# sisinflab/elliot

Measured on NVIDIA H100. Metric: bpr_triples_per_sec, higher is better.
Workload: dtype f32

## Files before the change

### elliot_b200/_lib.py

```python
import ctypes
import os

_HERE = os.path.dirname(os.path.abspath(__file__))
LIB_PATH = os.path.join(_HERE, "csrc", "libelliot_b200.so")

c_i32, c_i64, c_u64, c_f32, c_f64 = ctypes.c_int32, ctypes.c_int64, ctypes.c_uint64, ctypes.c_float, ctypes.c_double
c_int, c_void, c_size = ctypes.c_int, ctypes.c_void_p, ctypes.c_size_t

SIGNATURES = {
    "eb_last_error": (ctypes.c_char_p, []),
    "eb_version": (c_int, []),
    "eb_device_info": (c_int, [c_void, c_void]),
    "eb_bpr_step_f32": (c_int, [c_void, c_void, c_void, c_int, c_int, c_void, c_void, c_void, c_i64,
                                c_f32, c_f32, c_f32, c_f32, c_f32, c_void, c_int, c_void]),
    "eb_bpr_step_sampled_f32": (c_int, [c_void, c_void, c_void, c_int, c_int, c_i32, c_i32, c_void, c_void,
                                        c_i64, c_u64, c_u64, c_f32, c_f32, c_f32, c_f32, c_f32,
                                        c_void, c_void, c_void, c_void, c_void, c_size, c_int, c_void]),
    "eb_bpr_step_sampled_workspace_bytes": (c_size, [c_i64, c_i32]),
    "eb_bloom_build": (c_int, [c_void, c_void, c_i32, c_int, c_void, c_void]),
    "eb_bpr_step_sampled_filter_f32": (c_int, [c_void, c_void, c_void, c_int, c_int, c_i32, c_i32, c_void, c_void, c_void, c_int,
                                               c_i64, c_u64, c_u64, c_f32, c_f32, c_f32, c_f32, c_f32,
                                               c_void, c_void, c_void, c_void, c_void, c_size, c_int, c_void]),
    "eb_bpr_sample_philox_filter": (c_int, [c_i32, c_i32, c_void, c_void, c_void, c_int, c_i64, c_u64, c_u64, c_void, c_void, c_void,
                                            c_void]),
    "eb_bpr_sample_philox": (c_int, [c_i32, c_i32, c_void, c_void, c_i64, c_u64, c_u64, c_void, c_void, c_void,
                                     c_void]),
    "eb_bpr_step_host_f32": (c_int, [c_void, c_void, c_void, c_int, c_int, c_void, c_void, c_void, c_i64,
                                     c_f32, c_f32, c_f32, c_f32, c_f32, c_void, c_void, c_void, c_int, c_void]),
    "eb_bpr_step_host_packed_f32": (c_int, [c_void, c_void, c_void, c_int, c_int, c_void, c_i64, c_int, c_int,
                                            c_f32, c_f32, c_f32, c_f32, c_f32, c_void, c_void, c_void, c_int, c_void]),
    "eb_bpr_exact_workspace_bytes": (c_size, [c_i64, c_i32, c_i32]),
    "eb_bpr_exact_f64": (c_int, [c_void, c_void, c_void, c_int, c_int, c_i32, c_i32, c_void, c_void, c_void, c_i64,
                                 c_f64, c_f64, c_f64, c_f64, c_f64, c_void, c_void, c_size, c_void]),
    "eb_mt_seed": (c_int, [c_void, ctypes.c_uint32, c_void]),
    "eb_mt_sampler_workspace_bytes": (c_size, [c_i64]),
    "eb_mt_sampler_step": (c_int, [c_void, c_i32, c_i32, c_void, c_void, c_void, c_i64, c_void, c_void, c_void,
                                   c_void, c_size, c_void]),
    "eb_mt_raw": (c_int, [c_void, c_void, c_i64, c_void]),
    "eb_score_topk_workspace_bytes": (c_size, [c_i64, c_i32, c_int]),
    "eb_score_topk_f32": (c_int, [c_void, c_void, c_void, c_i32, c_int, c_int, c_void, c_void, c_void, c_i32, c_i64,
                                  c_int, c_void, c_void, c_void, c_size, c_void]),
    "eb_score_topk_f64": (c_int, [c_void, c_void, c_void, c_i32, c_int, c_int, c_void, c_void, c_void, c_i32, c_i64,
                                  c_int, c_void, c_void, c_void, c_size, c_void]),
    "eb_bpr_batch_grad_f32": (c_int, [c_void, c_void, c_void, c_void, c_void, c_void, c_int, c_int, c_void, c_void, c_void,
                                      c_i64, c_f32, c_f32, c_void, c_void]),
    "eb_adam_dense_f32": (c_int, [c_void, c_void, c_void, c_void, c_i64, c_f32, c_f32, c_f32, c_f32, c_i64, c_void]),
    "eb_adam_dense_copy_f32": (c_int, [c_void, c_void, c_void, c_void, c_i64, c_f32, c_f32, c_f32, c_f32, c_i64, c_void, c_void]),
    "eb_convert_bf16": (c_int, [c_void, c_int, c_int, c_i64, c_void, c_i64, c_int, c_void]),
    "eb_gemm_bf16_tn": (c_int, [c_void, c_i64, c_void, c_i64, c_void, c_i64, c_int, c_int, c_int, c_void, c_f32, c_int,
                                c_void]),
    "eb_gemm_bf16": (c_int, [c_void, c_i64, c_int, c_void, c_i64, c_int, c_void, c_i64, c_int, c_int, c_int, c_void, c_f32, c_int,
                             c_void]),
    "eb_gemm_bf16_out": (c_int, [c_void, c_i64, c_int, c_void, c_i64, c_int, c_void, c_i64, c_void, c_i64, c_int, c_int, c_int, c_void,
                                 c_f32, c_int, c_void]),
    "eb_gemm_f32_ref": (c_int, [c_void, c_i64, c_int, c_void, c_i64, c_int, c_void, c_i64, c_int, c_int, c_int, c_void, c_f32, c_int,
                                c_void]),
    "eb_vae_embed_fwd": (c_int, [c_void, c_void, c_int, c_void, c_void, c_void, c_int, c_void, c_i64, c_f32, c_u64, c_void]),
    "eb_vae_embed_bwd": (c_int, [c_void, c_int, c_void, c_void, c_void, c_int, c_void, c_i64, c_f32, c_u64, c_void]),
    "eb_vae_reparam_fwd": (c_int, [c_void, c_i64, c_int, c_int, c_void, c_i64, c_u64, c_u64, c_void, c_void]),
    "eb_vae_reparam_bwd": (c_int, [c_void, c_i64, c_int, c_int, c_void, c_i64, c_void, c_i64, c_u64, c_u64, c_f32, c_void]),
    "eb_vae_softmax": (c_int, [c_void, c_i64, c_int, c_void, c_void, c_void, c_int, c_void, c_void, c_int, c_void]),
    "eb_vae_softmax_bf16": (c_int, [c_void, c_i64, c_int, c_void, c_void, c_void, c_int, c_void, c_void, c_int, c_void, c_i64, c_void]),
    "eb_tanh_bwd": (c_int, [c_void, c_void, c_void, c_i64, c_void]),
    "eb_colsum": (c_int, [c_void, c_int, c_int, c_i64, c_void, c_void]),
    "eb_dense_topk_f32": (c_int, [c_void, c_i64, c_int, c_int, c_void, c_void, c_void, c_void, c_int, c_void, c_void, c_void]),
    "eb_neumf_gather": (c_int, [c_void, c_void, c_void, c_void, c_int, c_i64, c_void, c_void, c_i64, c_void, c_i64, c_void, c_i64, c_void]),
    "eb_neumf_head": (c_int, [c_void, c_i64, c_void, c_i64, c_int, c_void, c_void, c_void, c_i64, c_void, c_void, c_void, c_void,
                              c_void, c_void, c_void]),
    "eb_neumf_head_norm": (c_int, [c_void, c_i64, c_void, c_i64, c_int, c_void, c_void, c_void, c_i64, c_i64, c_void, c_void, c_void,
                                   c_void, c_void, c_void, c_void]),
    "eb_relu_bwd_copy": (c_int, [c_void, c_void, c_void, c_i64, c_void, c_void]),
    "eb_relu_bwd": (c_int, [c_void, c_void, c_void, c_i64, c_void]),
    "eb_neumf_scatter": (c_int, [c_void, c_void, c_int, c_i64, c_void, c_void, c_i64, c_void, c_i64, c_void, c_i64, c_void, c_void,
                                 c_void, c_void, c_void]),
    "eb_neumf_sample": (c_int, [c_i32, c_i32, c_void, c_void, c_int, c_u64, c_i64, c_void, c_void, c_void, c_void]),
    "eb_neumf_pair_h1": (c_int, [c_void, c_i64, c_void, c_i64, c_void, c_int, c_int, c_int, c_void, c_i64, c_void]),
    "eb_neumf_pair_h1_f32": (c_int, [c_void, c_i64, c_void, c_i64, c_void, c_int, c_int, c_int, c_void, c_i64, c_void]),
    "eb_neumf_pair_head": (c_int, [c_void, c_void, c_i64, c_int, c_int, c_int, c_int, c_void, c_i64, c_void, c_void, c_void, c_i64,
                                   c_void]),
    "eb_gather_rows_f32": (c_int, [c_void, c_i64, c_void, c_i64, c_int, c_void, c_i64, c_void]),
    "eb_scatter_add_rows_f32": (c_int, [c_void, c_i64, c_void, c_i64, c_int, c_void, c_i64, c_void]),
    "eb_bpr_step_rows_f32": (c_int, [c_void, c_i64, c_void, c_void, c_void, c_i64, c_i64, c_int, c_f32, c_f32, c_f32, c_f32, c_f32,
                                     c_void, c_void, c_void, c_void]),
    "eb_table_delta_f32": (c_int, [c_void, c_void, c_void, c_i64, c_void]),
    "eb_table_apply_delta_f32": (c_int, [c_void, c_void, c_void, c_i64, c_f32, c_void]),
    "eb_vae_step_workspace_bytes": (c_size, [c_int, c_int, c_int, c_int]),
    "eb_vae_train_step": (c_int, [c_void, c_void, c_int, c_f32, c_u64, c_u64, c_u64, c_f32, c_f32, c_void, c_void, c_size, c_int, c_void]),
    "eb_mf_pointwise_exact_f64": (c_int, [c_void, c_void, c_void, c_void, c_void, c_int, c_int, c_void, c_void, c_void, c_i64,
                                  c_f64, c_f64, c_i64, c_void, c_void]),
    "eb_mf_pointwise_step_f32": (c_int, [c_void, c_void, c_void, c_void, c_void, c_int, c_int, c_void, c_void, c_i64, c_int, c_i32,
                                 c_u64, c_u64, c_i64, c_i64, c_f32, c_f32, c_void, c_void, c_void, c_void, c_void, c_void]),
    "eb_eval_topk_workspace_bytes": (c_size, [c_i64, c_int]),
    "eb_eval_topk_f64": (c_int, [c_void, c_i64, c_int, c_int, c_void, c_void, c_void, c_void, c_void, c_void, c_void, c_void,
                         c_void, c_size, c_void]),
    "eb_partition_streams_create": (c_int, [c_int, c_int, ctypes.POINTER(ctypes.c_void_p), ctypes.POINTER(c_int)]),
    "eb_table_apply_delta_late_f32": (c_int, [c_void, c_void, c_void, c_void, c_i64, c_f32, c_void]),
    "eb_gmf_step_grads": (c_int, [c_void, c_void, c_i64, c_int, c_void, c_void, c_void, c_void, c_i64, c_i64, c_void, c_void, c_void,
                                  c_void, c_void]),
    "eb_gmf_scale_rows": (c_int, [c_void, c_i64, c_i64, c_int, c_void, c_void, c_i64, c_void]),
    "eb_sigmoid_inplace": (c_int, [c_void, c_i64, c_void]),
    "eb_pointwise_sample_philox": (c_int, [c_i32, c_i32, c_void, c_void, c_void, c_int, c_i64, c_u64, c_u64, c_void, c_void, c_void,
                                           c_void]),
    "eb_peer_alloc": (c_int, [c_size, ctypes.POINTER(ctypes.c_void_p)]),
    "eb_peer_free": (c_int, [c_void]),
    "eb_peer_export": (c_int, [c_void, c_void]),
# ... 81 lines not shown
```

### elliot_b200/csrc/bpr_train.cu

```cuda
#include <cooperative_groups.h>
#include <cub/cub.cuh>
#include <stdlib.h>

#include <type_traits>

#include "bpr_update.cuh"

namespace eb {

struct HogwildParams {
    float *U, *V, *b;
    int ld;
    const int32_t *tu, *ti, *tj;
    int64_t n;
    BprHyper hp;
    double *loss;
    int32_t n_users, n_items;
    const int64_t *indptr;
    const int32_t *indices;
    uint64_t seed, first;
    int32_t *out_u, *out_i, *out_j;
    float *Vp[EB_MAX_PEERS], *bp[EB_MAX_PEERS];
    ShardMap shards;
    const uint32_t *filter;
// ... 529 lines not shown

template <int DP, bool SAMPLE, bool ATOMIC, bool PEER, bool ROUNDS>
static int launch_hogwild_t(const HogwildParams &p, int reserve_sms, cudaStream_t st) {
    auto kern = bpr_hogwild_kernel<DP, SAMPLE, ATOMIC, PEER, ROUNDS>;
    unsigned grid;
    if (int rc = persistent_grid((const void *)kern, 0, p.n, reserve_sms, grid)) return rc;
    if (ROUNDS) {
        void *args[] = {const_cast<HogwildParams *>(&p)};
        EB_CUDA(cudaLaunchCooperativeKernel((const void *)kern, dim3(grid), dim3(256), args, 0, st));
    } else {
        kern<<<grid, 256, 0, st>>>(p);
    }
    EB_CUDA(cudaGetLastError());
    return EB_OK;
}

template <int... DPS, class F>
static int with_stride(int dp, const char *strides, F &&f) {
    int rc = EB_OK;
    const bool found = ((dp == DPS && (rc = f(std::integral_constant<int, DPS>{}), true)) || ...);
    return found ? rc : set_err(EB_ERR_ARG, "row stride ld=%d must be one of %s", dp, strides);
}

static void item_table_l2_window(const HogwildParams &p, cudaStream_t st) {
    static const int env = [] { const char *e = getenv("EB_L2_PERSIST"); return e ? atoi(e) : 0; }();
    if (!env || !p.V) return;
    static int max_persist = -1, max_window = 0;
    if (max_persist < 0) {
        int dev = 0; cudaGetDevice(&dev);
        cudaDeviceGetAttribute(&max_persist, cudaDevAttrMaxPersistingL2CacheSize, dev);
        cudaDeviceGetAttribute(&max_window, cudaDevAttrMaxAccessPolicyWindowSize, dev);
    }
    const size_t bytes = (size_t)p.n_items * (size_t)p.ld * sizeof(float);
    if (max_persist <= 0 || bytes > (size_t)max_persist || bytes > (size_t)max_window) return;
    static size_t carved = 0;
    if (carved != bytes) { cudaDeviceSetLimit(cudaLimitPersistingL2CacheSize, bytes); carved = bytes; }
    cudaStreamAttrValue attr{};
    attr.accessPolicyWindow.base_ptr = (void *)p.V;
    attr.accessPolicyWindow.num_bytes = bytes;
    attr.accessPolicyWindow.hitRatio = 1.0f;
    attr.accessPolicyWindow.hitProp = cudaAccessPropertyPersisting;
    attr.accessPolicyWindow.missProp = env == 2 ? cudaAccessPropertyNormal : cudaAccessPropertyStreaming;
    cudaStreamSetAttribute(st, cudaStreamAttributeAccessPolicyWindow, &attr);
}

template <int DP, bool ATOMIC>
static int launch_grouped_t(const HogwildParams &p, int reserve_sms, cudaStream_t st) {
    auto kern = bpr_grouped_kernel<DP, ATOMIC>;
    unsigned grid;
    if (int rc = persistent_grid((const void *)kern, 0, p.n, reserve_sms, grid)) return rc;
    kern<<<grid, 256, 0, st>>>(p);
    EB_CUDA(cudaGetLastError());
    return EB_OK;
}

static inline size_t align_up(size_t x, size_t a = 256) { return (x + a - 1) / a * a; }

static int bits_for(uint64_t v) { int b = 1; while ((v >> b) != 0) b++; return b; }

constexpr int64_t GROUP_MAX = (int64_t)INT32_MAX;

struct GroupLayout {
    size_t key_a, key_b, val_a, val_b, cub, cub_bytes, total;
};

static GroupLayout group_layout(int64_t n, int32_t n_users) {
    const int64_t m = n < GROUP_MAX ? n : GROUP_MAX;
    GroupLayout L;
    size_t off = 0;
    L.key_a = off; off += align_up(sizeof(uint32_t) * (size_t)m);
    L.key_b = off; off += align_up(sizeof(uint32_t) * (size_t)m);
    L.val_a = off; off += align_up(sizeof(int32_t) * (size_t)m);
    L.val_b = off; off += align_up(sizeof(int32_t) * (size_t)m);
    cub::DoubleBuffer<uint32_t> keys(nullptr, nullptr);
    cub::DoubleBuffer<int32_t> vals(nullptr, nullptr);
    size_t cb = 0;
    cub::DeviceRadixSort::SortPairs(nullptr, cb, keys, vals, (int)m, 0, bits_for((uint64_t)n_users));
    L.cub_bytes = cb;
    L.cub = off; off += align_up(cb);
    L.total = off;
    return L;
}

template <int DP, bool ATOMIC>
static int launch_grouped(HogwildParams p, int reserve, char *ws, const GroupLayout &L, cudaStream_t st) {
    const int ubits = bits_for((uint64_t)p.n_users);
    const int64_t n = p.n;
    const uint64_t first = p.first;
    int32_t *out_u = p.out_u, *out_i = p.out_i, *out_j = p.out_j;
    int sms = sm_count() - reserve;
    if (sms < 1) sms = 1;
    for (int64_t c0 = 0; c0 < n; c0 += GROUP_MAX) {
        p.n = n - c0 < GROUP_MAX ? n - c0 : GROUP_MAX;
        p.first = first + (uint64_t)c0;
        if (out_u) { p.out_u = out_u + c0; p.out_i = out_i + c0; p.out_j = out_j + c0; }
        cub::DoubleBuffer<uint32_t> keys((uint32_t *)(ws + L.key_a), (uint32_t *)(ws + L.key_b));
        cub::DoubleBuffer<int32_t> vals((int32_t *)(ws + L.val_a), (int32_t *)(ws + L.val_b));
        int64_t grid = (p.n + 255) / 256;
        if (grid > (int64_t)sms * 8) grid = (int64_t)sms * 8;
        user_key_kernel<<<(unsigned)grid, 256, 0, st>>>(p, keys.Current(), vals.Current());
        EB_CUDA(cudaGetLastError());
        size_t cb = L.cub_bytes;
        EB_CUDA(cub::DeviceRadixSort::SortPairs(ws + L.cub, cb, keys, vals, (int)p.n, 0, ubits, st));
        p.order = vals.Current();
        if (int rc = launch_grouped_t<DP, ATOMIC>(p, reserve, st)) return rc;
    }
    return EB_OK;
}

template <bool SAMPLE>
static int launch_hogwild(const HogwildParams &p, int dp, int flags, cudaStream_t st, void *ws = nullptr, size_t ws_bytes = 0) {
    const bool atomic = !(flags & 1);
    const bool rounds = (flags & 64) != 0;
    const int reserve = (flags >> 8) & 0xff;
    EB_ARG(!(flags & 32), "the shared-memory-staged kernel exists for sharded item tables only");
    EB_ARG(atomic || !rounds, "deterministic rounds run with atomic updates");
    if constexpr (SAMPLE) {
        if (!rounds) {
            const GroupLayout L = group_layout(p.n, p.n_users);
            if (!ws || ws_bytes < L.total) return set_err(EB_ERR_WORKSPACE, "workspace %zu < required %zu", ws ? ws_bytes : 0, L.total);
            return with_stride<8, 16, 32, 64, 128, 256>(dp, "8,16,32,64,128,256 floats", [&](auto dpc) {
                constexpr int DP = decltype(dpc)::value;
                item_table_l2_window(p, st);
                return atomic ? launch_grouped<DP, true>(p, reserve, (char *)ws, L, st)
                              : launch_grouped<DP, false>(p, reserve, (char *)ws, L, st);
            });
        }
    }
    item_table_l2_window(p, st);
    return with_stride<8, 16, 32, 64, 128, 256>(dp, "8,16,32,64,128,256 floats", [&](auto dpc) {
        constexpr int DP = decltype(dpc)::value;
        if constexpr (!SAMPLE) {
            if (!rounds) return atomic ? launch_hogwild_t<DP, false, true, false, false>(p, reserve, st)
                                       : launch_hogwild_t<DP, false, false, false, false>(p, reserve, st);
        }
        return launch_hogwild_t<DP, SAMPLE, true, false, true>(p, reserve, st);
    });
}

template <bool SAMPLE>
static int launch_hogwild_peer(const HogwildParams &p, int dp, int flags, cudaStream_t st) {
    const int reserve = (flags >> 8) & 0xff;
    EB_ARG(!(flags & 64), "deterministic rounds exist for local tables only (other GPUs update peer rows concurrently)");
    const bool stage = !(flags & (1 | 16));
    return with_stride<32, 64, 128>(dp, "32,64,128 floats for sharded item tables", [&](auto dpc) {
        constexpr int DP = decltype(dpc)::value;
        return stage ? launch_stage_t<DP, SAMPLE>(p, reserve, st) : launch_hogwild_t<DP, SAMPLE, true, true, false>(p, reserve, st);
    });
}

static int fill_peer(HogwildParams &p, float *const *V_shards, float *const *b_shards, int n_shards, int32_t shard_rows,
                     int32_t n_items) {
    EB_ARG(V_shards && b_shards && n_shards >= 1 && n_shards <= EB_MAX_PEERS, "1 <= n_shards <= %d", EB_MAX_PEERS);
    EB_ARG(shard_rows >= 1 && (int64_t)shard_rows * n_shards >= n_items, "shards do not cover the item range");
    for (int s = 0; s < n_shards; s++) {
        EB_ARG(V_shards[s] && b_shards[s] && ((uintptr_t)V_shards[s] % 16) == 0, "null / misaligned shard pointer %d", s);
        p.Vp[s] = V_shards[s]; p.bp[s] = b_shards[s];
    }
    for (int s = n_shards; s < EB_MAX_PEERS; s++) { p.Vp[s] = V_shards[0]; p.bp[s] = b_shards[0]; }
    p.shards = shard_map(shard_rows);
    return EB_OK;
}

static int check_tables(const void *U, const void *V, const void *b, int d, int ld) {
    EB_ARG(U && V && b, "null table pointer");
    EB_ARG(d >= 1 && ld >= d, "need 1 <= d <= ld (d=%d ld=%d)", d, ld);
    EB_ARG(((uintptr_t)U % 16) == 0 && ((uintptr_t)V % 16) == 0, "tables must be 16-byte aligned");
    return EB_OK;
}

struct ExactParams {
    double *U, *V, *b;
    int d, ld;
    const int32_t *tu, *ti, *tj;
    const int32_t *ku, *ki, *kj;
    int32_t *cntU, *cntI, *ticket;
    int64_t n;
    double lr, reg_u, reg_b, reg_pos, reg_neg;
    double *loss;
};

__device__ __forceinline__ int ld_acquire(const int32_t *p) {
    int v;
    asm volatile("ld.acquire.gpu.global.s32 %0, [%1];" : "=r"(v) : "l"(p) : "memory");
    return v;
}
__device__ __forceinline__ void st_release(int32_t *p, int v) {
    asm volatile("st.release.gpu.global.s32 [%0], %1;" ::"l"(p), "r"(v) : "memory");
}

template <int NE>
__global__ void __launch_bounds__(128) bpr_exact_kernel(const ExactParams p) {
    const int lane = threadIdx.x & 31;
    double loss_acc = 0.0;
    for (;;) {
        int t = 0;
        if (lane == 0) t = atomicAdd(p.ticket, 1);
        t = __shfl_sync(0xffffffffu, t, 0);
        if (t >= p.n) break;
        const int u = __ldg(p.tu + t), i = __ldg(p.ti + t), j = __ldg(p.tj + t);
        const int wu = __ldg(p.ku + t), wi = __ldg(p.ki + t), wj = __ldg(p.kj + t);
        int32_t *cu = p.cntU + u, *ci = p.cntI + i, *cj = p.cntI + j;
        {
            unsigned ns = 8;
            for (;;) {
                const bool ready = (ld_acquire(cu) == wu) & (ld_acquire(ci) == wi) & (ld_acquire(cj) == wj);
                if (__all_sync(0xffffffffu, ready)) break;
                __nanosleep(ns);
                if (ns < 128) ns <<= 1;
            }
        }
        double *pu = p.U + (int64_t)u * p.ld, *pi = p.V + (int64_t)i * p.ld, *pj = p.V + (int64_t)j * p.ld;
        double a[NE], vi[NE], vj[NE];
        double xi = 0.0, xj = 0.0;
#pragma unroll
        for (int e = 0; e < NE; e++) {
            const int k = lane + 32 * e;
            a[e] = 0.0; vi[e] = 0.0; vj[e] = 0.0;
            if (k < p.d) {
// ... 82 lines not shown
    L.cnt = off; off += align_up(sizeof(int32_t) * ((size_t)n_users + (size_t)n_items + 64));
    size_t cb = 0;
    cub::DeviceRadixSort::SortKeys(nullptr, cb, (const uint64_t *)nullptr, (uint64_t *)nullptr, (int64_t)(2 * n), 0, 64);
    L.cub_bytes = cb;
    L.cub = off; off += align_up(cb);
    L.total = off;
    return L;
}

}

using namespace eb;

extern "C" int eb_bpr_step_f32(float *U, float *V, float *item_bias, int d, int ld, const int32_t *tu,
                               const int32_t *ti, const int32_t *tj, int64_t n, float lr, float reg_u, float reg_b,
                               float reg_pos, float reg_neg, double *loss, int flags, void *stream) {
    if (int rc = check_tables(U, V, item_bias, d, ld)) return rc;
    EB_ARG(n >= 0, "n < 0");
    if (n == 0) return EB_OK;
    EB_ARG(tu && ti && tj, "null triple arrays");
    HogwildParams p{};
    p.U = U; p.V = V; p.b = item_bias; p.ld = ld; p.tu = tu; p.ti = ti; p.tj = tj; p.n = n;
    p.hp = {lr, reg_u, reg_b, reg_pos, reg_neg}; p.loss = loss;
    return launch_hogwild<false>(p, ld, flags, (cudaStream_t)stream);
}

static int set_filter(HogwildParams &p, const uint32_t *filter, int filter_words) {
    if (!filter) return EB_OK;
    EB_ARG(filter_words >= 1 && filter_words <= 1024 && (filter_words & (filter_words - 1)) == 0,
           "filter_words must be a power of two in [1, 1024] (got %d)", filter_words);
    int lb = 5;
    while ((1 << (lb - 5)) < filter_words) lb++;
    p.filter = filter; p.filter_log2bits = lb;
    return EB_OK;
}

extern "C" int eb_bloom_build(const int64_t *csr_indptr, const int32_t *csr_indices, int32_t n_users, int filter_words,
                              uint32_t *out, void *stream) {
    EB_ARG(csr_indptr && csr_indices && out && n_users >= 1, "bad argument");
    HogwildParams p{};
    if (int rc = set_filter(p, out, filter_words)) return rc;
    int64_t grid = ((int64_t)n_users * 32 + 255) / 256;
    const int64_t cap = (int64_t)sm_count() * 8;
    if (grid > cap) grid = cap;
    bloom_build_kernel<<<(unsigned)grid, 256, 0, (cudaStream_t)stream>>>(csr_indptr, csr_indices, n_users, p.filter_log2bits, out);
    EB_CUDA(cudaGetLastError());
    return EB_OK;
}

extern "C" int eb_bpr_step_sampled_f32(float *U, float *V, float *item_bias, int d, int ld, int32_t n_users,
                                       int32_t n_items, const int64_t *csr_indptr, const int32_t *csr_indices,
                                       int64_t n, uint64_t seed, uint64_t first_triple, float lr, float reg_u,
                                       float reg_b, float reg_pos, float reg_neg, double *loss, int32_t *out_u,
                                       int32_t *out_i, int32_t *out_j, void *workspace, size_t workspace_bytes, int flags,
                                       void *stream) {
    return eb_bpr_step_sampled_filter_f32(U, V, item_bias, d, ld, n_users, n_items, csr_indptr, csr_indices, nullptr, 0, n, seed,
                                          first_triple, lr, reg_u, reg_b, reg_pos, reg_neg, loss, out_u, out_i, out_j, workspace,
                                          workspace_bytes, flags, stream);
}

extern "C" size_t eb_bpr_step_sampled_workspace_bytes(int64_t n, int32_t n_users) {
    if (n <= 0 || n_users <= 0) return 256;
    return group_layout(n, n_users).total;
}

extern "C" int eb_bpr_step_sampled_filter_f32(float *U, float *V, float *item_bias, int d, int ld, int32_t n_users,
                                              int32_t n_items, const int64_t *csr_indptr, const int32_t *csr_indices,
                                              const uint32_t *filter, int filter_words, int64_t n, uint64_t seed,
                                              uint64_t first_triple, float lr, float reg_u, float reg_b, float reg_pos,
                                              float reg_neg, double *loss, int32_t *out_u, int32_t *out_i, int32_t *out_j,
                                              void *workspace, size_t workspace_bytes, int flags, void *stream) {
    if (int rc = check_tables(U, V, item_bias, d, ld)) return rc;
    EB_ARG(n >= 0 && n_users > 0 && n_items > 1, "bad sizes");
    EB_ARG(csr_indptr && csr_indices, "null CSR");
    EB_ARG((!out_u && !out_i && !out_j) || (out_u && out_i && out_j), "out_u/out_i/out_j: all or none");
    if (n == 0) return EB_OK;
    HogwildParams p{};
    p.U = U; p.V = V; p.b = item_bias; p.ld = ld; p.n = n;
    p.hp = {lr, reg_u, reg_b, reg_pos, reg_neg}; p.loss = loss;
    p.n_users = n_users; p.n_items = n_items; p.indptr = csr_indptr; p.indices = csr_indices;
    p.seed = seed; p.first = first_triple; p.out_u = out_u; p.out_i = out_i; p.out_j = out_j;
    if (int rc = set_filter(p, filter, filter_words)) return rc;
    return launch_hogwild<true>(p, ld, flags, (cudaStream_t)stream, workspace, workspace_bytes);
}

extern "C" int eb_bpr_step_peer_f32(float *U, float *const *V_shards, float *const *b_shards, int n_shards, int32_t shard_rows,
                                    int d, int ld, int32_t n_items, const int32_t *tu, const int32_t *ti, const int32_t *tj, int64_t n,
                                    float lr, float reg_u, float reg_b, float reg_pos, float reg_neg, double *loss, int flags,
                                    void *stream) {
    EB_ARG(U && d >= 1 && ld >= d && ((uintptr_t)U % 16) == 0, "bad user table");
    EB_ARG(n >= 0, "n < 0");
    HogwildParams p{};
    if (int rc = fill_peer(p, V_shards, b_shards, n_shards, shard_rows, n_items)) return rc;
    if (n == 0) return EB_OK;
    EB_ARG(tu && ti && tj, "null triple arrays");
    p.U = U; p.ld = ld; p.tu = tu; p.ti = ti; p.tj = tj; p.n = n;
    p.hp = {lr, reg_u, reg_b, reg_pos, reg_neg}; p.loss = loss;
    return launch_hogwild_peer<false>(p, ld, flags, (cudaStream_t)stream);
}

extern "C" int eb_bpr_step_sampled_peer_f32(float *U, float *const *V_shards, float *const *b_shards, int n_shards, int32_t shard_rows,
                                            int d, int ld, int32_t n_users, int32_t n_items, const int64_t *csr_indptr,
                                            const int32_t *csr_indices, const uint32_t *filter, int filter_words, int64_t n,
                                            uint64_t seed, uint64_t first_triple, float lr,
                                            float reg_u, float reg_b, float reg_pos, float reg_neg, double *loss, int32_t *out_u,
                                            int32_t *out_i, int32_t *out_j, int flags, void *stream) {
    EB_ARG(U && d >= 1 && ld >= d && ((uintptr_t)U % 16) == 0, "bad user table");
    EB_ARG(n >= 0 && n_users > 0 && n_items > 1, "bad sizes");
    EB_ARG(csr_indptr && csr_indices, "null CSR");
    EB_ARG((!out_u && !out_i && !out_j) || (out_u && out_i && out_j), "out_u/out_i/out_j: all or none");
    HogwildParams p{};
    if (int rc = fill_peer(p, V_shards, b_shards, n_shards, shard_rows, n_items)) return rc;
    if (n == 0) return EB_OK;
    p.U = U; p.ld = ld; p.n = n;
    p.hp = {lr, reg_u, reg_b, reg_pos, reg_neg}; p.loss = loss;
    p.n_users = n_users; p.n_items = n_items; p.indptr = csr_indptr; p.indices = csr_indices;
    p.seed = seed; p.first = first_triple; p.out_u = out_u; p.out_i = out_i; p.out_j = out_j;
    p.no_item_updates = (flags >> 2) & 1;
    if (int rc = set_filter(p, filter, filter_words)) return rc;
    return launch_hogwild_peer<true>(p, ld, flags, (cudaStream_t)stream);
}

extern "C" int eb_bpr_sample_philox(int32_t n_users, int32_t n_items, const int64_t *csr_indptr,
                                    const int32_t *csr_indices, int64_t n, uint64_t seed, uint64_t first_triple,
                                    int32_t *out_u, int32_t *out_i, int32_t *out_j, void *stream) {
    return eb_bpr_sample_philox_filter(n_users, n_items, csr_indptr, csr_indices, nullptr, 0, n, seed, first_triple, out_u, out_i,
                                       out_j, stream);
}

extern "C" int eb_bpr_sample_philox_filter(int32_t n_users, int32_t n_items, const int64_t *csr_indptr,
                                           const int32_t *csr_indices, const uint32_t *filter, int filter_words, int64_t n,
                                           uint64_t seed, uint64_t first_triple, int32_t *out_u, int32_t *out_i, int32_t *out_j,
                                           void *stream) {
    EB_ARG(n >= 0 && n_users > 0 && n_items > 1, "bad sizes");
    EB_ARG(csr_indptr && csr_indices && out_u && out_i && out_j, "null pointer");
    if (n == 0) return EB_OK;
    HogwildParams p{};
    p.n = n; p.n_users = n_users; p.n_items = n_items; p.indptr = csr_indptr; p.indices = csr_indices;
    p.seed = seed; p.first = first_triple; p.out_u = out_u; p.out_i = out_i; p.out_j = out_j;
    if (int rc = set_filter(p, filter, filter_words)) return rc;
    int64_t grid = (n + 255) / 256;
    int64_t cap = (int64_t)sm_count() * 8;
    if (grid > cap) grid = cap;
    philox_sample_kernel<<<(unsigned)grid, 256, 0, (cudaStream_t)stream>>>(p);
    EB_CUDA(cudaGetLastError());
    return EB_OK;
}

extern "C" int eb_pointwise_sample_philox(int32_t n_users, int32_t n_items, const int64_t *csr_indptr, const int32_t *csr_indices,
                                          const uint32_t *filter, int filter_words, int64_t n, uint64_t seed, uint64_t first,
                                          int32_t *out_u, int32_t *out_i, float *out_label, void *stream) {
    EB_ARG(n >= 0 && n_users > 0 && n_items > 1, "bad sizes");
    EB_ARG(csr_indptr && csr_indices && out_u && out_i && out_label, "null pointer");
    if (n == 0) return EB_OK;
    HogwildParams p{};
    p.n = n; p.n_users = n_users; p.n_items = n_items; p.indptr = csr_indptr; p.indices = csr_indices;
    p.seed = seed; p.first = first; p.out_u = out_u; p.out_i = out_i;
    if (int rc = set_filter(p, filter, filter_words)) return rc;
    int64_t grid = (n + 255) / 256;
    const int64_t cap = (int64_t)sm_count() * 8;
    if (grid > cap) grid = cap;
    pointwise_sample_kernel<<<(unsigned)grid, 256, 0, (cudaStream_t)stream>>>(p, out_label);
    EB_CUDA(cudaGetLastError());
    return EB_OK;
}

// ... 99 lines not shown
```

### elliot_b200/ops.py

```python
import ctypes

import torch

from ._lib import check, lib

F32_STRIDES = (8, 16, 32, 64, 128, 256)


def padded_dim(d):
    for s in F32_STRIDES:
        if d <= s:
            return s
    raise ValueError(f"factors={d} > 256 is not supported by the fp32 kernels")


def _ptr(t):
    return 0 if t is None else t.data_ptr()


def _stream(t):
    return torch.cuda.current_stream(t.device).cuda_stream


def _need_cuda(*ts):
    for t in ts:
        if t is not None and not t.is_cuda:
            raise RuntimeError("elliot_b200 ops need CUDA tensors (no CPU fallback exists)")


def _chk_idx(*ts):
    for t in ts:
        if t.dtype != torch.int32 or not t.is_contiguous():
            raise TypeError("index tensors must be contiguous int32")


def device_info():
    sm = ctypes.c_int(0); cc = ctypes.c_int(0)
    check(lib().eb_device_info(ctypes.byref(sm), ctypes.byref(cc)))
    return sm.value, cc.value


def bpr_step_f32(U, V, b, d, tu, ti, tj, lr, reg_u, reg_b, reg_pos, reg_neg, loss=None, racy=False, deterministic=False):
    _need_cuda(U, V, b, tu, ti, tj, loss)
    _chk_idx(tu, ti, tj)
    assert U.dtype == torch.float32 and V.dtype == torch.float32 and b.dtype == torch.float32
    assert U.stride(1) == 1 and V.stride(1) == 1 and U.stride(0) == V.stride(0)
    with torch.cuda.device(U.device):
        check(lib().eb_bpr_step_f32(_ptr(U), _ptr(V), _ptr(b), d, U.stride(0), _ptr(tu), _ptr(ti), _ptr(tj), tu.numel(),
                                    lr, reg_u, reg_b, reg_pos, reg_neg, _ptr(loss), (1 if racy else 0) | (64 if deterministic else 0),
                                    _stream(U)))


def bloom_build(indptr, indices, n_users, words=32):
    _need_cuda(indptr, indices)
    assert indptr.dtype == torch.int64 and indices.dtype == torch.int32
    out = torch.empty((n_users, words), dtype=torch.int32, device=indptr.device)
    with torch.cuda.device(indptr.device):
        check(lib().eb_bloom_build(_ptr(indptr), _ptr(indices), n_users, words, _ptr(out), _stream(indptr)))
    return out


def bpr_step_sampled_f32(U, V, b, d, n_users, n_items, indptr, indices, n, seed, first, lr, reg_u, reg_b, reg_pos,
                         reg_neg, loss=None, out=None, racy=False, reserve_sms=0, filter=None, deterministic=False, _variant=0):
    _need_cuda(U, V, b, indptr, indices, loss, filter)
    assert indptr.dtype == torch.int64 and indices.dtype == torch.int32
    ou = oi = oj = None
    if out is not None:
        ou, oi, oj = out
        _need_cuda(ou, oi, oj); _chk_idx(ou, oi, oj)
    ws = None
    if not deterministic:
        ws = _ws_grouped.get(lib().eb_bpr_step_sampled_workspace_bytes(n, n_users), U.device)
    with torch.cuda.device(U.device):
        check(lib().eb_bpr_step_sampled_filter_f32(_ptr(U), _ptr(V), _ptr(b), d, U.stride(0), n_users, n_items, _ptr(indptr),
                                                   _ptr(indices), _ptr(filter), 0 if filter is None else filter.shape[1], n, seed,
                                                   first, lr, reg_u, reg_b, reg_pos, reg_neg, _ptr(loss), _ptr(ou), _ptr(oi),
                                                   _ptr(oj), _ptr(ws), 0 if ws is None else ws.numel(),
                                                   (1 if racy else 0) | (64 if deterministic else 0) | ((int(reserve_sms) & 0xff) << 8) | int(_variant),
                                                   _stream(U)))


def bpr_sample_philox(n_users, n_items, indptr, indices, n, seed, first=0, filter=None):
    _need_cuda(indptr, indices, filter)
    dev = indptr.device
    u = torch.empty(n, dtype=torch.int32, device=dev); i = torch.empty_like(u); j = torch.empty_like(u)
    with torch.cuda.device(dev):
        check(lib().eb_bpr_sample_philox_filter(n_users, n_items, _ptr(indptr), _ptr(indices), _ptr(filter),
                                                0 if filter is None else filter.shape[1], n, seed, first, _ptr(u), _ptr(i), _ptr(j),
                                                _stream(indptr)))
    return u, i, j


def bpr_step_host_f32(U, V, b, d, tu_host, ti_host, tj_host, lr, reg_u, reg_b, reg_pos, reg_neg, staging, loss_dev,
                      loss_host, racy=False, sync=True, reserve_sms=0):
    _need_cuda(U, V, b, staging, loss_dev)
    n = tu_host.numel()
    assert not tu_host.is_cuda and tu_host.dtype == torch.int32 and staging.numel() >= 3 * n
    with torch.cuda.device(U.device):
        check(lib().eb_bpr_step_host_f32(_ptr(U), _ptr(V), _ptr(b), d, U.stride(0), _ptr(tu_host), _ptr(ti_host),
                                         _ptr(tj_host), n, lr, reg_u, reg_b, reg_pos, reg_neg, _ptr(staging),
                                         _ptr(loss_dev), _ptr(loss_host), (1 if racy else 0) | (0 if sync else 2) | ((int(reserve_sms) & 0xff) << 8),
                                         _stream(U)))


def pack_bits(n_users, n_items):
    bu, bi = max(1, (int(n_users) - 1).bit_length()), max(1, (int(n_items) - 1).bit_length())
    if bu + 2 * bi > 64:
        raise ValueError("ids too wide for the packed 64-bit triple format")
    return bu, bi


def pack_triples(tu, ti, tj, n_users, n_items):
    bu, bi = pack_bits(n_users, n_items)
    return tu.to(torch.int64) | (ti.to(torch.int64) << bu) | (tj.to(torch.int64) << (bu + bi))


def bpr_step_host_packed_f32(U, V, b, d, packed_host, n_users, n_items, lr, reg_u, reg_b, reg_pos, reg_neg, staging, loss_dev,
                             loss_host, sync=True, reserve_sms=0):
    _need_cuda(U, V, b, staging, loss_dev)
    n = packed_host.numel()
    assert not packed_host.is_cuda and packed_host.dtype == torch.int64 and staging.dtype == torch.int64 and staging.numel() >= n
    bu, bi = pack_bits(n_users, n_items)
    with torch.cuda.device(U.device):
        check(lib().eb_bpr_step_host_packed_f32(_ptr(U), _ptr(V), _ptr(b), d, U.stride(0), _ptr(packed_host), n, bu, bi,
                                                lr, reg_u, reg_b, reg_pos, reg_neg, _ptr(staging), _ptr(loss_dev), _ptr(loss_host),
                                                (0 if sync else 2) | ((int(reserve_sms) & 0xff) << 8), _stream(U)))


class _Workspace:

    def __init__(self):
        self.buf = None

    def get(self, nbytes, device):
        if self.buf is None or self.buf.numel() < nbytes or self.buf.device != device:
            self.buf = torch.empty(max(int(nbytes), 256), dtype=torch.uint8, device=device)
        return self.buf


_ws_exact, _ws_sampler, _ws_score, _ws_grouped = _Workspace(), _Workspace(), _Workspace(), _Workspace()


def bpr_exact_f64(U, V, b, d, tu, ti, tj, lr, reg_u, reg_b, reg_pos, reg_neg, loss=None):
    _need_cuda(U, V, b, tu, ti, tj, loss)
    _chk_idx(tu, ti, tj)
    assert U.dtype == torch.float64 and V.dtype == torch.float64 and b.dtype == torch.float64
    n = tu.numel()
    nu, ni = U.shape[0], V.shape[0]
    nbytes = lib().eb_bpr_exact_workspace_bytes(n, nu, ni)
    ws = _ws_exact.get(nbytes, U.device)
    with torch.cuda.device(U.device):
        check(lib().eb_bpr_exact_f64(_ptr(U), _ptr(V), _ptr(b), d, U.stride(0), nu, ni, _ptr(tu), _ptr(ti), _ptr(tj), n,
                                     lr, reg_u, reg_b, reg_pos, reg_neg, _ptr(loss), _ptr(ws), ws.numel(), _stream(U)))


class MtSampler:

    def __init__(self, n_users, n_items, indptr, set_indices, sorted_indices, seed=42):
        _need_cuda(indptr, set_indices, sorted_indices)
        assert indptr.dtype == torch.int64 and set_indices.dtype == torch.int32 and sorted_indices.dtype == torch.int32
        self.n_users, self.n_items = n_users, n_items
        self.indptr, self.set_indices, self.sorted_indices = indptr, set_indices, sorted_indices
# ... 820 lines not shown
```

### include/elliot_b200.h

```cpp
#ifndef ELLIOT_B200_H
#define ELLIOT_B200_H

#include <stddef.h>
#include <stdint.h>

#ifdef __cplusplus
extern "C" {
#endif

#define EB_OK 0
#define EB_ERR_ARG (-1)
#define EB_ERR_CUDA (-2)
#define EB_ERR_WORKSPACE (-3)
#define EB_ERR_DATA (-4)

const char *eb_last_error(void);
int eb_version(void);
int eb_device_info(int *sm_count, int *cc);


int eb_bpr_step_f32(float *U, float *V, float *item_bias, int d, int ld,
                    const int32_t *tu, const int32_t *ti, const int32_t *tj, int64_t n,
                    float lr, float reg_u, float reg_b, float reg_pos, float reg_neg,
                    double *loss, int flags, void *stream);

size_t eb_bpr_step_sampled_workspace_bytes(int64_t n, int32_t n_users);
int eb_bpr_step_sampled_f32(float *U, float *V, float *item_bias, int d, int ld,
                            int32_t n_users, int32_t n_items,
                            const int64_t *csr_indptr, const int32_t *csr_indices,
                            int64_t n, uint64_t seed, uint64_t first_triple,
                            float lr, float reg_u, float reg_b, float reg_pos, float reg_neg,
                            double *loss, int32_t *out_u, int32_t *out_i, int32_t *out_j,
                            void *workspace, size_t workspace_bytes, int flags, void *stream);

int eb_bloom_build(const int64_t *csr_indptr, const int32_t *csr_indices, int32_t n_users, int filter_words,
                   uint32_t *out, void *stream);
int eb_bpr_step_sampled_filter_f32(float *U, float *V, float *item_bias, int d, int ld,
                                   int32_t n_users, int32_t n_items,
                                   const int64_t *csr_indptr, const int32_t *csr_indices,
                                   const uint32_t *filter, int filter_words,
                                   int64_t n, uint64_t seed, uint64_t first_triple,
                                   float lr, float reg_u, float reg_b, float reg_pos, float reg_neg,
                                   double *loss, int32_t *out_u, int32_t *out_i, int32_t *out_j,
                                   void *workspace, size_t workspace_bytes, int flags, void *stream);
int eb_bpr_sample_philox_filter(int32_t n_users, int32_t n_items, const int64_t *csr_indptr,
                                const int32_t *csr_indices, const uint32_t *filter, int filter_words, int64_t n,
                                uint64_t seed, uint64_t first_triple, int32_t *out_u, int32_t *out_i, int32_t *out_j,
                                void *stream);

int eb_bpr_sample_philox(int32_t n_users, int32_t n_items,
                         const int64_t *csr_indptr, const int32_t *csr_indices,
                         int64_t n, uint64_t seed, uint64_t first_triple,
                         int32_t *out_u, int32_t *out_i, int32_t *out_j, void *stream);

int eb_bpr_step_host_f32(float *U, float *V, float *item_bias, int d, int ld,
                         const int32_t *tu_host, const int32_t *ti_host, const int32_t *tj_host, int64_t n,
                         float lr, float reg_u, float reg_b, float reg_pos, float reg_neg,
                         int32_t *staging, double *loss_dev, double *loss_host, int flags, void *stream);
int eb_bpr_step_host_packed_f32(float *U, float *V, float *item_bias, int d, int ld, const uint64_t *packed_host, int64_t n,
                                int bits_u, int bits_i, float lr, float reg_u, float reg_b, float reg_pos, float reg_neg,
                                uint64_t *staging, double *loss_dev, double *loss_host, int flags, void *stream);

size_t eb_bpr_exact_workspace_bytes(int64_t n, int32_t n_users, int32_t n_items);
int eb_bpr_exact_f64(double *U, double *V, double *item_bias, int d, int ld,
                     int32_t n_users, int32_t n_items,
                     const int32_t *tu, const int32_t *ti, const int32_t *tj, int64_t n,
                     double lr, double reg_u, double reg_b, double reg_pos, double reg_neg,
                     double *loss, void *workspace, size_t workspace_bytes, void *stream);

int eb_mt_seed(uint32_t *state, uint32_t seed, void *stream);
size_t eb_mt_sampler_workspace_bytes(int64_t events);
int eb_mt_sampler_step(uint32_t *state, int32_t n_users, int32_t n_items,
                       const int64_t *indptr, const int32_t *set_indices, const int32_t *sorted_indices,
                       int64_t events, int32_t *out_u, int32_t *out_i, int32_t *out_j,
                       void *workspace, size_t workspace_bytes, void *stream);
int eb_mt_raw(uint32_t *state, uint32_t *out, int64_t n, void *stream);

size_t eb_score_topk_workspace_bytes(int64_t n_sel, int32_t n_items, int elem_size);
int eb_score_topk_f32(const float *U, const float *V, const float *item_bias, int32_t n_items, int d, int ld,
                      const int64_t *mask_indptr, const int32_t *mask_indices,
                      const int32_t *users, int32_t user_begin, int64_t n_sel, int k,
                      int32_t *out_idx, float *out_val, void *workspace, size_t workspace_bytes, void *stream);
int eb_score_topk_f64(const double *U, const double *V, const double *item_bias, int32_t n_items, int d, int ld,
                      const int64_t *mask_indptr, const int32_t *mask_indices,
                      const int32_t *users, int32_t user_begin, int64_t n_sel, int k,
                      int32_t *out_idx, double *out_val, void *workspace, size_t workspace_bytes, void *stream);

int eb_bpr_batch_grad_f32(const float *Gu, const float *Gi, const float *Bi, float *dGu, float *dGi, float *dBi,
                          int d, int ld, const int32_t *tu, const int32_t *ti, const int32_t *tj, int64_t n,
                          float l_w, float l_b, double *loss, void *stream);
int eb_adam_dense_f32(float *var, float *m, float *v, float *grad, int64_t n, float lr, float beta1, float beta2,
                      float eps, int64_t step, void *stream);
int eb_adam_dense_copy_f32(float *var, float *m, float *v, float *grad, int64_t n, float lr, float beta1, float beta2,
                           float eps, int64_t step, void *copy_bf16, void *stream);

int eb_vae_embed_fwd(const float *W1, const float *b1, int H, const int64_t *indptr, const int32_t *indices,
                     const int32_t *rows, int B, float *h1, int64_t ldh, float drop_rate, uint64_t seed, void *stream);
int eb_vae_embed_bwd(float *dW1, int H, const int64_t *indptr, const int32_t *indices, const int32_t *rows, int B,
                     const float *dpre1, int64_t ldd, float drop_rate, uint64_t seed, void *stream);
int eb_vae_reparam_fwd(const float *ml, int64_t ldml, int B, int L, float *z, int64_t ldz, uint64_t seed, uint64_t step,
                       double *kl_sum, void *stream);
int eb_vae_reparam_bwd(const float *ml, int64_t ldml, int B, int L, const float *dz, int64_t lddz, float *dml,
                       int64_t lddml, uint64_t seed, uint64_t step, float anneal, void *stream);
int eb_vae_softmax(float *logits, int64_t ld, int n_items, const int64_t *indptr, const int32_t *indices,
                   const int32_t *rows, int B, double *nll_sum, float *lse_out, int write_grad, void *stream);
int eb_vae_softmax_bf16(float *logits, int64_t ld, int n_items, const int64_t *indptr, const int32_t *indices,
                        const int32_t *rows, int B, double *nll_sum, float *lse_out, int write_grad, void *grad_bf16,
                        int64_t ld_bf16, void *stream);
int eb_tanh_bwd(const float *dout, const float *out, float *dpre, int64_t n, void *stream);
int eb_colsum(const float *src, int rows, int cols, int64_t ld, float *out, void *stream);
typedef struct eb_vae_model {
    int n_items, H, L, reserved;
    float *W1, *b1, *W2, *b2, *W3, *b3, *W4, *b4;
    float *gW1, *gb1, *gW2, *gb2, *gW3, *gb3, *gW4, *gb4;
    float *mW1, *mb1, *mW2, *mb2, *mW3, *mb3, *mW4, *mb4;
    float *vW1, *vb1, *vW2, *vb2, *vW3, *vb3, *vW4, *vb4;
    void *W2b, *W3b, *W4b, *W2t, *W3t, *W4t;
    const int64_t *indptr;
    const int32_t *indices;
} eb_vae_model;
size_t eb_vae_step_workspace_bytes(int n_items, int H, int L, int B);
int eb_vae_train_step(const eb_vae_model *m, const int32_t *rows, int B, float drop_rate, uint64_t noise_seed,
                      uint64_t drop_seed, uint64_t step, float anneal, float lr, double *acc, void *workspace,
                      size_t workspace_bytes, int phase, void *stream);
int eb_dense_topk_f32(float *scores, int64_t ld, int n_rows, int n_items, const int64_t *mask_indptr,
                      const int32_t *mask_indices, const int32_t *rows, const float *shift, int k, int32_t *out_idx,
                      float *out_val, void *stream);
// ... 174 lines not shown
```

Baseline: 2.298 billion.

## Prefetch next step's user-sorted schedule on a side stream

Result: faster. 2.443 billion, median of 6 (+6.3%).

```diff
diff --git a/elliot_b200/_lib.py b/elliot_b200/_lib.py
--- a/elliot_b200/_lib.py
+++ b/elliot_b200/_lib.py
@@ -21,6 +21,11 @@
     "eb_bpr_step_sampled_filter_f32": (c_int, [c_void, c_void, c_void, c_int, c_int, c_i32, c_i32, c_void, c_void, c_void, c_int,
                                                c_i64, c_u64, c_u64, c_f32, c_f32, c_f32, c_f32, c_f32,
                                                c_void, c_void, c_void, c_void, c_void, c_size, c_int, c_void]),
+    "eb_bpr_schedule_sampled": (c_int, [c_i32, c_i32, c_void, c_i64, c_u64, c_u64, c_void, c_size, ctypes.POINTER(c_size), c_int,
+                                        c_void]),
+    "eb_bpr_apply_sampled_filter_f32": (c_int, [c_void, c_void, c_void, c_int, c_int, c_i32, c_i32, c_void, c_void, c_void, c_int,
+                                                c_i64, c_u64, c_u64, c_f32, c_f32, c_f32, c_f32, c_f32,
+                                                c_void, c_void, c_void, c_void, c_void, c_int, c_void]),
     "eb_bpr_sample_philox_filter": (c_int, [c_i32, c_i32, c_void, c_void, c_void, c_int, c_i64, c_u64, c_u64, c_void, c_void, c_void,
                                             c_void]),
     "eb_bpr_sample_philox": (c_int, [c_i32, c_i32, c_void, c_void, c_i64, c_u64, c_u64, c_void, c_void, c_void,
diff --git a/elliot_b200/csrc/bpr_train.cu b/elliot_b200/csrc/bpr_train.cu
--- a/elliot_b200/csrc/bpr_train.cu
+++ b/elliot_b200/csrc/bpr_train.cu
@@ -635,27 +635,32 @@
     return L;
 }
 
+static int schedule_grouped(const HogwildParams &p, int reserve, char *ws, const GroupLayout &L, cudaStream_t st,
+                            const int32_t *&order) {
+    int sms = sm_count() - reserve;
+    if (sms < 1) sms = 1;
+    cub::DoubleBuffer<uint32_t> keys((uint32_t *)(ws + L.key_a), (uint32_t *)(ws + L.key_b));
+    cub::DoubleBuffer<int32_t> vals((int32_t *)(ws + L.val_a), (int32_t *)(ws + L.val_b));
+    int64_t grid = (p.n + 255) / 256;
+    if (grid > (int64_t)sms * 8) grid = (int64_t)sms * 8;
+    user_key_kernel<<<(unsigned)grid, 256, 0, st>>>(p, keys.Current(), vals.Current());
+    EB_CUDA(cudaGetLastError());
+    size_t cb = L.cub_bytes;
+    EB_CUDA(cub::DeviceRadixSort::SortPairs(ws + L.cub, cb, keys, vals, (int)p.n, 0, bits_for((uint64_t)p.n_users), st));
+    order = vals.Current();
+    return EB_OK;
+}
+
 template <int DP, bool ATOMIC>
 static int launch_grouped(HogwildParams p, int reserve, char *ws, const GroupLayout &L, cudaStream_t st) {
-    const int ubits = bits_for((uint64_t)p.n_users);
     const int64_t n = p.n;
     const uint64_t first = p.first;
     int32_t *out_u = p.out_u, *out_i = p.out_i, *out_j = p.out_j;
-    int sms = sm_count() - reserve;
-    if (sms < 1) sms = 1;
     for (int64_t c0 = 0; c0 < n; c0 += GROUP_MAX) {
         p.n = n - c0 < GROUP_MAX ? n - c0 : GROUP_MAX;
         p.first = first + (uint64_t)c0;
         if (out_u) { p.out_u = out_u + c0; p.out_i = out_i + c0; p.out_j = out_j + c0; }
-        cub::DoubleBuffer<uint32_t> keys((uint32_t *)(ws + L.key_a), (uint32_t *)(ws + L.key_b));
-        cub::DoubleBuffer<int32_t> vals((int32_t *)(ws + L.val_a), (int32_t *)(ws + L.val_b));
-        int64_t grid = (p.n + 255) / 256;
-        if (grid > (int64_t)sms * 8) grid = (int64_t)sms * 8;
-        user_key_kernel<<<(unsigned)grid, 256, 0, st>>>(p, keys.Current(), vals.Current());
-        EB_CUDA(cudaGetLastError());
-        size_t cb = L.cub_bytes;
-        EB_CUDA(cub::DeviceRadixSort::SortPairs(ws + L.cub, cb, keys, vals, (int)p.n, 0, ubits, st));
-        p.order = vals.Current();
+        if (int rc = schedule_grouped(p, reserve, ws, L, st, p.order)) return rc;
         if (int rc = launch_grouped_t<DP, ATOMIC>(p, reserve, st)) return rc;
     }
     return EB_OK;
@@ -688,6 +693,17 @@
                                        : launch_hogwild_t<DP, false, false, false, false>(p, reserve, st);
         }
         return launch_hogwild_t<DP, SAMPLE, true, false, true>(p, reserve, st);
+    });
+}
+
+static int launch_apply(const HogwildParams &p, int dp, int flags, cudaStream_t st) {
+    const bool atomic = !(flags & 1);
+    const int reserve = (flags >> 8) & 0xff;
+    EB_ARG(!(flags & (32 | 64)), "the grouped update runs free-running on local tables (no rounds, no staged kernel)");
+    return with_stride<8, 16, 32, 64, 128, 256>(dp, "8,16,32,64,128,256 floats", [&](auto dpc) {
+        constexpr int DP = decltype(dpc)::value;
+        item_table_l2_window(p, st);
+        return atomic ? launch_grouped_t<DP, true>(p, reserve, st) : launch_grouped_t<DP, false>(p, reserve, st);
     });
 }
 
@@ -936,6 +952,44 @@
     p.seed = seed; p.first = first_triple; p.out_u = out_u; p.out_i = out_i; p.out_j = out_j;
     if (int rc = set_filter(p, filter, filter_words)) return rc;
     return launch_hogwild<true>(p, ld, flags, (cudaStream_t)stream, workspace, workspace_bytes);
+}
+
+extern "C" int eb_bpr_schedule_sampled(int32_t n_users, int32_t n_items, const int64_t *csr_indptr, int64_t n, uint64_t seed,
+                                       uint64_t first_triple, void *workspace, size_t workspace_bytes, size_t *order_offset,
+                                       int flags, void *stream) {
+    EB_ARG(n >= 1 && n <= GROUP_MAX && n_users > 0 && n_items > 1, "bad sizes (a schedule covers 1..%lld triples)",
+           (long long)GROUP_MAX);
+    EB_ARG(csr_indptr && order_offset, "null pointer");
+    const GroupLayout L = group_layout(n, n_users);
+    if (!workspace || workspace_bytes < L.total)
+        return set_err(EB_ERR_WORKSPACE, "workspace %zu < required %zu", workspace ? workspace_bytes : 0, L.total);
+    HogwildParams p{};
+    p.n = n; p.n_users = n_users; p.n_items = n_items; p.indptr = csr_indptr; p.seed = seed; p.first = first_triple;
+    const int32_t *order = nullptr;
+    if (int rc = schedule_grouped(p, (flags >> 8) & 0xff, (char *)workspace, L, (cudaStream_t)stream, order)) return rc;
+    *order_offset = (size_t)((const char *)order - (const char *)workspace);
+    return EB_OK;
+}
+
+extern "C" int eb_bpr_apply_sampled_filter_f32(float *U, float *V, float *item_bias, int d, int ld, int32_t n_users,
+                                               int32_t n_items, const int64_t *csr_indptr, const int32_t *csr_indices,
+                                               const uint32_t *filter, int filter_words, int64_t n, uint64_t seed,
+                                               uint64_t first_triple, float lr, float reg_u, float reg_b, float reg_pos,
+                                               float reg_neg, double *loss, int32_t *out_u, int32_t *out_i, int32_t *out_j,
+                                               const int32_t *order, int flags, void *stream) {
+    if (int rc = check_tables(U, V, item_bias, d, ld)) return rc;
+    EB_ARG(n >= 1 && n <= GROUP_MAX && n_users > 0 && n_items > 1, "bad sizes (an apply covers 1..%lld triples)",
+           (long long)GROUP_MAX);
+    EB_ARG(csr_indptr && csr_indices && order, "null CSR or order");
+    EB_ARG((!out_u && !out_i && !out_j) || (out_u && out_i && out_j), "out_u/out_i/out_j: all or none");
+    HogwildParams p{};
+    p.U = U; p.V = V; p.b = item_bias; p.ld = ld; p.n = n;
+    p.hp = {lr, reg_u, reg_b, reg_pos, reg_neg}; p.loss = loss;
+    p.n_users = n_users; p.n_items = n_items; p.indptr = csr_indptr; p.indices = csr_indices;
+    p.seed = seed; p.first = first_triple; p.out_u = out_u; p.out_i = out_i; p.out_j = out_j;
+    p.order = order;
+    if (int rc = set_filter(p, filter, filter_words)) return rc;
+    return launch_apply(p, ld, flags, (cudaStream_t)stream);
 }
 
 extern "C" int eb_bpr_step_peer_f32(float *U, float *const *V_shards, float *const *b_shards, int n_shards, int32_t shard_rows,
diff --git a/elliot_b200/ops.py b/elliot_b200/ops.py
--- a/elliot_b200/ops.py
+++ b/elliot_b200/ops.py
@@ -1,4 +1,5 @@
 import ctypes
+import os
 
 import torch
 
@@ -68,16 +69,105 @@
     if out is not None:
         ou, oi, oj = out
         _need_cuda(ou, oi, oj); _chk_idx(ou, oi, oj)
+    flags = (1 if racy else 0) | (64 if deterministic else 0) | ((int(reserve_sms) & 0xff) << 8) | int(_variant)
+    fw = 0 if filter is None else filter.shape[1]
+    if _prefetch_on and not deterministic and not _variant and 1 <= n <= _SCHEDULE_MAX:
+        with torch.cuda.device(U.device):
+            _schedules_of(U.device).step(U, V, b, d, n_users, n_items, indptr, indices, filter, fw, n, seed, first,
+                                         (lr, reg_u, reg_b, reg_pos, reg_neg), loss, (ou, oi, oj), flags)
+        return
     ws = None
     if not deterministic:
         ws = _ws_grouped.get(lib().eb_bpr_step_sampled_workspace_bytes(n, n_users), U.device)
     with torch.cuda.device(U.device):
         check(lib().eb_bpr_step_sampled_filter_f32(_ptr(U), _ptr(V), _ptr(b), d, U.stride(0), n_users, n_items, _ptr(indptr),
-                                                   _ptr(indices), _ptr(filter), 0 if filter is None else filter.shape[1], n, seed,
+                                                   _ptr(indices), _ptr(filter), fw, n, seed,
                                                    first, lr, reg_u, reg_b, reg_pos, reg_neg, _ptr(loss), _ptr(ou), _ptr(oi),
-                                                   _ptr(oj), _ptr(ws), 0 if ws is None else ws.numel(),
-                                                   (1 if racy else 0) | (64 if deterministic else 0) | ((int(reserve_sms) & 0xff) << 8) | int(_variant),
-                                                   _stream(U)))
+                                                   _ptr(oj), _ptr(ws), 0 if ws is None else ws.numel(), flags, _stream(U)))
+
+
+_SCHEDULE_MAX = 2**31 - 1
+_prefetch_on = os.environ.get("EB_BPR_PREFETCH", "1") != "0"
+_schedules = {}
+
+
+def set_bpr_prefetch(enabled):
+    global _prefetch_on
+    was, _prefetch_on = _prefetch_on, bool(enabled)
+    if not enabled:
+        for s in _schedules.values():
+            s.release()
+        _schedules.clear()
+    return was
+
+
+def _schedules_of(device):
+    i = device.index if device.index is not None else torch.cuda.current_device()
+    if i not in _schedules:
+        _schedules[i] = _Schedules(torch.device("cuda", i))
+    return _schedules[i]
+
+
+class _Schedules:
+
+    def __init__(self, device):
+        self.device = device
+        self.side = torch.cuda.Stream(device)
+        self.buf = [None, None]
+        self.off = [0, 0]
+        self.key = [None, None]
+        self.built = [torch.cuda.Event(), torch.cuda.Event()]
+        self.read = [torch.cuda.Event(), torch.cuda.Event()]
+        self.ready = torch.cuda.Event()
+        self.cur = 0
+        self.last = None
+
+    def release(self):
+        for e in self.built + self.read:
+            e.synchronize()
+        self.buf = [None, None]
+        self.key = [None, None]
+
+    def _schedule(self, s, n_users, n_items, indptr, n, seed, first, flags, stream):
+        need = int(lib().eb_bpr_step_sampled_workspace_bytes(n, n_users))
+        if self.buf[s] is None or self.buf[s].numel() < need:
+            self.built[s].synchronize(); self.read[s].synchronize()
+            self.buf[s] = None
+            self.buf[s] = torch.empty(need, dtype=torch.uint8, device=self.device)
+            self.buf[s].record_stream(self.side)
+        off = ctypes.c_size_t(0)
+        check(lib().eb_bpr_schedule_sampled(n_users, n_items, _ptr(indptr), n, seed, first, _ptr(self.buf[s]), self.buf[s].numel(),
+                                            ctypes.byref(off), flags & 0xff00, stream.cuda_stream))
+        self.off[s] = off.value
+
+    def step(self, U, V, b, d, n_users, n_items, indptr, indices, filt, fw, n, seed, first, hp, loss, out, flags):
+        st = torch.cuda.current_stream(self.device)
+        csr = (n_users, n_items, indptr.data_ptr(), indices.data_ptr(), _ptr(filt), indptr._version, indices._version)
+        key = (seed, first, n) + csr
+        s = 0 if self.key[0] == key else 1 if self.key[1] == key else None
+        if s is None:
+            s = self.cur
+            st.wait_event(self.built[s]); st.wait_event(self.read[s])
+            self._schedule(s, n_users, n_items, indptr, n, seed, first, flags, st)
+        else:
+            st.wait_event(self.built[s])
+        self.key[s] = None
+        ahead = self.last == (first - n, n)
+        if ahead:
+            self.ready.record(st)
+        order = self.buf[s].data_ptr() + self.off[s]
+        check(lib().eb_bpr_apply_sampled_filter_f32(_ptr(U), _ptr(V), _ptr(b), d, U.stride(0), n_users, n_items, _ptr(indptr),
+                                                    _ptr(indices), _ptr(filt), fw, n, seed, first, *hp, _ptr(loss),
+                                                    *(_ptr(x) for x in out), order, flags, st.cuda_stream))
+        self.read[s].record(st)
+        self.cur, self.last = s, (first, n)
+        if ahead:
+            o = 1 - s
+            self.side.wait_event(self.ready); self.side.wait_event(self.read[o])
+            self._schedule(o, n_users, n_items, indptr, n, seed, first + n, flags, self.side)
+            self.built[o].record(self.side)
+            indptr.record_stream(self.side)
+            self.key[o] = (seed, first + n, n) + csr
 
 
 def bpr_sample_philox(n_users, n_items, indptr, indices, n, seed, first=0, filter=None):
diff --git a/include/elliot_b200.h b/include/elliot_b200.h
--- a/include/elliot_b200.h
+++ b/include/elliot_b200.h
@@ -43,6 +43,17 @@
                                    float lr, float reg_u, float reg_b, float reg_pos, float reg_neg,
                                    double *loss, int32_t *out_u, int32_t *out_i, int32_t *out_j,
                                    void *workspace, size_t workspace_bytes, int flags, void *stream);
+int eb_bpr_schedule_sampled(int32_t n_users, int32_t n_items, const int64_t *csr_indptr, int64_t n, uint64_t seed,
+                            uint64_t first_triple, void *workspace, size_t workspace_bytes, size_t *order_offset, int flags,
+                            void *stream);
+int eb_bpr_apply_sampled_filter_f32(float *U, float *V, float *item_bias, int d, int ld,
+                                    int32_t n_users, int32_t n_items,
+                                    const int64_t *csr_indptr, const int32_t *csr_indices,
+                                    const uint32_t *filter, int filter_words,
+                                    int64_t n, uint64_t seed, uint64_t first_triple,
+                                    float lr, float reg_u, float reg_b, float reg_pos, float reg_neg,
+                                    double *loss, int32_t *out_u, int32_t *out_i, int32_t *out_j,
+                                    const int32_t *order, int flags, void *stream);
 int eb_bpr_sample_philox_filter(int32_t n_users, int32_t n_items, const int64_t *csr_indptr,
                                 const int32_t *csr_indices, const uint32_t *filter, int filter_words, int64_t n,
                                 uint64_t seed, uint64_t first_triple, int32_t *out_u, int32_t *out_i, int32_t *out_j,
```
